# shaneson0/attacking_federate_learning

Measured on AMD Instinct MI355X. Metric: aggregation rounds/sec at N clients x D params (Bulyan), higher is better.
Workload: dtype f32 (Gram: fp16x2 split of every fp32 operand, 3 fp16 MFMAs per block, fp32/fp64 accumulate; <= 2e-7 of |gi||gj| vs f...

## Files before the change

attacking_federate_learning_amd/_native.py:

```python
import ctypes
import os

_HERE = os.path.dirname(os.path.abspath(__file__))
LIB_PATH = os.environ.get('BYZ_LIBRARY') or os.path.join(_HERE, 'libbyzagg.so')

OK, E_INVALID, E_PRECONDITION, E_HIP, E_UNSUPPORTED, E_NO_WINNER, E_COLLECTIVE = 0, -1, -2, -3, -4, -5, -6

KERNELS = ('column_stats', 'gram_tile', 'gram_reduce', 'distances', 'row_sort', 'krum_argmin',
           'bulyan_loop', 'trimmed_mean', 'misc', 'plane_split')

c_i64, c_i32, c_int, c_f32, c_vp = ctypes.c_int64, ctypes.c_int32, ctypes.c_int, ctypes.c_float, ctypes.c_void_p
_P = ctypes.POINTER



class GeomedParams(ctypes.Structure):
    _fields_ = [('nu', ctypes.c_double), ('max_iter', c_i64), ('ftol', ctypes.c_double)]


class CclipParams(ctypes.Structure):
    _fields_ = [('tau', ctypes.c_double), ('iters', c_i64)]


class DncParams(ctypes.Structure):
# ... 90 lines not shown
    'byz_robust_lr_info': [c_vp, _P(c_i64)],
    'byz_robust_lr_host': [c_vp, c_vp, c_i64, c_i64, c_i64, c_vp, c_vp],
    'byz_bucket_means_dev': [c_vp, c_vp, c_i64, c_i64, c_i64, c_vp, c_i64, c_vp, c_i64, c_vp],
    'byz_bucket_means_host': [c_vp, c_vp, c_i64, c_i64, c_vp, c_i64, c_vp],
    'byz_dnc_scores_dev': [c_vp, c_vp, c_i64, c_i64, c_i64, c_vp, c_i64, c_i64, c_vp, c_vp],
    'byz_dnc_select_dev': [c_vp, c_vp, c_i64, c_i64, c_i64, _P(DncParams), c_vp, c_vp, c_vp, c_vp],
    'byz_dnc_dev': [c_vp, c_vp, c_i64, c_i64, c_i64, _P(DncParams), c_vp, c_vp, c_vp, c_vp],
    'byz_dnc_info': [c_vp, _P(c_i64), _P(c_i64)],
    'byz_dnc_host': [c_vp, c_vp, c_i64, c_i64, _P(DncParams), c_vp, c_vp, c_vp, _P(c_i64)],
    'byz_dnc_sharded_dev': [c_vp, c_vp, c_i64, c_i64, c_i64, _P(DncParams), c_vp, c_vp, c_vp, c_vp, c_vp, c_vp, c_vp],
    'byz_timing_enable': [c_vp, c_int],
    'byz_timing_reset': [c_vp],
    'byz_timing_read': [c_vp, c_int, _P(ctypes.c_double), _P(c_i64)],
    'byz_kernel_name': [c_int],
    'byz_selftest_lane_exchange_dev': [c_vp, c_vp, _P(c_i32), c_vp],
}
_RESTYPES = {'byz_last_error': ctypes.c_char_p, 'byz_kernel_name': ctypes.c_char_p, 'byz_ctx_destroy': None}

ALLREDUCE_F64_FN = ctypes.CFUNCTYPE(c_int, c_vp, c_vp, c_i64, c_vp)

EXPORTED_SYMBOLS = tuple(_PROTOTYPES)

_lib = None


class NativeLibraryMissing(RuntimeError):
    pass


def _share_hip_runtime_with_torch():
# ... 43 lines not shown
```

attacking_federate_learning_amd/csrc/api.hip:

```cpp
#include "common.hpp"

#include <cstring>

namespace byz {

static thread_local char g_error[1024] = "";

void set_error(const char* fmt, ...) {
    va_list ap;
    va_start(ap, fmt);
    vsnprintf(g_error, sizeof(g_error), fmt, ap);
    va_end(ap);
}

namespace {

int64_t python_prefix_len(int64_t length, int64_t stop) {
    if (stop >= 0) return stop < length ? stop : length;
    return length + stop > 0 ? length + stop : 0;
}

int enter(byz_ctx* ctx) {
    if (!ctx) {
        set_error("null context");
// ... 1621 lines not shown
        (void)hipEventDestroy(ev.first);
        (void)hipEventDestroy(ev.second);
    }
    slot.pending.clear();
    if (total_ms) *total_ms = slot.total_ms;
    if (launches) *launches = slot.launches;
    return BYZ_OK;
}

int byz_selftest_lane_exchange_dev(byz_ctx* ctx, int32_t* out_dev, int32_t* n_patterns_host, void* stream) {
    BYZ_TRY(enter(ctx));
    BYZ_REQUIRE(out_dev && n_patterns_host, "selftest: bad arguments");
    return launch_lane_selftest(ctx, out_dev, n_patterns_host, as_stream(stream));
}

}
```

attacking_federate_learning_amd/csrc/common.hpp:

```cpp
#pragma once

#include <hip/hip_runtime.h>

#include <cstdarg>
#include <cstdint>
#include <cstdio>
#include <cstdlib>
#include <string>
#include <unordered_map>
#include <vector>

#include "../../include/byzagg.h"

namespace byz {

void set_error(const char* fmt, ...);

#define BYZ_HIP(expr)                                                                       \
    do {                                                                                    \
        hipError_t e_ = (expr);                                                             \
        if (e_ != hipSuccess) {                                                             \
            ::byz::set_error("%s failed: %s (%s:%d)", #expr, hipGetErrorString(e_), __FILE__, \
                             __LINE__);                                                     \
            return BYZ_E_HIP;                                                               \
// ... 69 lines not shown
    int num_cus = 256;
    byz::Buffer gram_partials;
    byz::Buffer gram;
    byz::Buffer tile_order;
    byz::Buffer dup_rep;
    byz::Buffer gram_tickets;
    byz::Buffer gram_planes;
    byz::Buffer gram_chunk_sums;
    byz::Buffer plane_unscale;
    byz::Buffer plane_order;
    byz::Buffer spec_owner;
    byz::Buffer split_redo;
    std::vector<int32_t> plane_order_host;
    int64_t plane_order_T = -1;
    int64_t plane_order_share = 1 * 65536 + 0;
    byz::Buffer row_signature;
    byz::Buffer unique_rows;
    byz::Buffer row_map;
    byz::Buffer gram_compact;
    std::vector<int32_t> tile_order_host;
    int64_t tile_order_T = -1;
    int64_t tile_order_share = 1 * 65536 + 0;
    byz::Buffer tile_owned;
    int64_t row_map_rows = 0;
    byz::Buffer gram_rep;
    byz::Buffer near_pairs;
    byz::Buffer near_sq;
    byz::Buffer near_rows;
    byz::Buffer near_partial;
    int64_t near_pair_capacity = 0;
// ... 151 lines not shown
                         int64_t n, float lr, float z, float* out, hipStream_t stream);
int launch_assemble_row(byz_ctx* ctx, float* row, int64_t n_cols, int64_t n_segments, const float* const* segments,
                        const int64_t* lengths, hipStream_t stream);
int launch_assemble_columns(byz_ctx* ctx, float* G, int64_t n_rows, int64_t n_cols, int64_t ld, int64_t n_segments,
                            const float* const* segments, const int64_t* lengths, hipStream_t stream);
int launch_assemble_rows_again(byz_ctx* ctx, float* G, int64_t n_cols, int64_t ld, int64_t n_clients, int64_t n_segments,
                               hipStream_t stream);
int launch_assemble_rows(byz_ctx* ctx, float* G, int64_t n_cols, int64_t ld, int64_t n_clients, int64_t n_segments,
                         const float* const* segments, const int64_t* lengths, hipStream_t stream);

int launch_gram(byz_ctx* ctx, const float* G, int64_t n_rows, int64_t n_cols, int64_t ld, double* gram,
                hipStream_t stream);
bool gram_planes_enabled();
int launch_gram_planes(byz_ctx* ctx, const float* G, int64_t n_rows, int64_t n_cols, int64_t ld, const int32_t* row_index,
                       double* slabs, int share_count, int share_index, uint8_t* owned_host, bool f16, hipStream_t stream);
int launch_gram_share(byz_ctx* ctx, const float* G, int64_t n_rows, int64_t n_cols, int64_t ld, const int32_t* row_index,
                      int share_count, int share_index, double* gram, hipStream_t stream, bool accumulate = false);
int find_unique_rows(byz_ctx* ctx, const float* G, int64_t n_rows, int64_t n_cols, int64_t ld, hipStream_t stream,
                     int64_t* n_unique_host);
int launch_gram_expand(byz_ctx* ctx, const double* compact, int64_t n_unique, int64_t n_rows, double* gram,
                       hipStream_t stream);
int launch_distances_from_gram(byz_ctx* ctx, const double* gram, int64_t n, float* dist, hipStream_t stream,
                               const float* G, int64_t n_cols, int64_t ld);
int launch_near_pair_sqdist(byz_ctx* ctx, const float* G, int64_t n_cols, int64_t ld, const int32_t* row_index,
                            double* sq_dev, hipStream_t stream);
int launch_near_pair_apply(byz_ctx* ctx, const double* sq_dev, int64_t n, float* dist, hipStream_t stream);

int launch_row_sort(byz_ctx* ctx, const float* dist, int64_t n, int64_t prefix_len, int64_t drop_count,
                    bool want_tables, hipStream_t stream);
int launch_krum_argmin(byz_ctx* ctx, int64_t n, int32_t* winner_dev, hipStream_t stream);
// ... 77 lines not shown
```

attacking_federate_learning_amd/csrc/gram_planes.hip:

```cpp
#include "common.hpp"

#include <cstring>
#include <type_traits>

namespace byz {
namespace {

constexpr int kWgRows = 256;
constexpr int kWgCols = 128;
constexpr int kSlab = 128;
constexpr int kThreads = 512;
constexpr int kFragBytes = 1024;
constexpr int kRowBlocks = (kWgRows + kWgCols) / 32;
constexpr int kChunkCols = 8192;
constexpr int kChunkSteps = kChunkCols / 16;
constexpr int kFlushSteps = 16;
constexpr int kSpareRoundsPercent = 10;

typedef float f32x16 __attribute__((ext_vector_type(16)));
typedef float f32x4 __attribute__((ext_vector_type(4)));
typedef __bf16 bf16x8 __attribute__((ext_vector_type(8)));
typedef _Float16 f16x8 __attribute__((ext_vector_type(8)));
typedef uint32_t u32x4 __attribute__((ext_vector_type(4)));

// ... 518 lines not shown
    }
    asm volatile("s_waitcnt vmcnt(0)" ::: "memory");
    __syncthreads();
    if (tid == 0) {
        __builtin_amdgcn_fence(__ATOMIC_RELEASE, "agent");
        asm volatile("s_waitcnt vmcnt(0)" ::: "memory");
        __hip_atomic_store(tickets + t_list, chunk + 1, __ATOMIC_RELAXED, __HIP_MEMORY_SCOPE_AGENT);
        __hip_atomic_fetch_add(done, 1, __ATOMIC_RELAXED, __HIP_MEMORY_SCOPE_AGENT);
    }
}

template <int NBUF, bool DEFER>
__global__ __launch_bounds__(512, 1) void gram_planes16_kernel(const u32x4* __restrict__ planes, int64_t n_steps,
                                                            const double* __restrict__ unscale, int64_t rows_pad,
                                                            double* __restrict__ partial, int n_tiles,
                                                            const int2* __restrict__ tile_order, int n_chunks,
                                                            int* __restrict__ tickets, int round_size, int run, int t128,
                                                            int slab_live0, int n_blocks32,
                                                            int32_t* __restrict__ device_status,
                                                            float* __restrict__ chunk_sums,
                                                            float* __restrict__ ragged_sums) {
    constexpr int PLANES = 2;
    constexpr int kRbBytes = PLANES * kFragBytes;
    constexpr int kStage = kRowBlocks * kRbBytes;
    constexpr int NW = 8;
    constexpr int kPerWave = kRowBlocks * PLANES / NW;
    constexpr int kSuperFlush = kFlushSteps / 2;
    static_assert(kRowBlocks * PLANES % NW == 0 && NBUF == 6, "ring arithmetic below");
    typedef f16x8 frag_t;
    extern __shared__ __attribute__((aligned(16))) unsigned char lds[];

    const int xcd = blockIdx.x & 7;
    const int seq = blockIdx.x >> 3;
// ... 23 lines not shown
            while (v <= 0) {
                __builtin_amdgcn_s_sleep(1);
                v = __hip_atomic_load(slot, __ATOMIC_RELAXED, __HIP_MEMORY_SCOPE_AGENT);
            }
            claimed_round = v - 1;
        }
        __syncthreads();
    }
    const int unit = __builtin_amdgcn_readfirstlane(claimed_round * run + seq % run);
    const int chunk = __builtin_amdgcn_readfirstlane(unit / n_tiles);
    if (chunk >= n_chunks) {
        if (threadIdx.x == 0) __hip_atomic_fetch_add(done, 1, __ATOMIC_RELAXED, __HIP_MEMORY_SCOPE_AGENT);
        return;
    }
    const int t_list = unit - chunk * n_tiles;
    const int2 tt = tile_order[t_list];
    const int bi = __builtin_amdgcn_readfirstlane(tt.x);
    const int tj = __builtin_amdgcn_readfirstlane(tt.y);

    const int tid = threadIdx.x;
    const int lane = tid & 63;
    const int wave = __builtin_amdgcn_readfirstlane(tid >> 6);
    const int wr = wave >> 1, wc = wave & 1;
    const int ti = 2 * bi + wr / 2;
    const int row_in_slab = (wr % 2) * 64;
    unsigned live_blocks = 0;
    if (tj <= ti && ti < t128 && n_blocks32 < 0) {
        live_blocks = 15u;
    } else if (tj <= ti && ti < t128) {
#pragma unroll
        for (int m = 0; m < 2; ++m)
#pragma unroll
            for (int n = 0; n < 2; ++n) {
                const int rblk = ti * 4 + row_in_slab / 32 + m, cblk = tj * 4 + wc * 2 + n;
                if (rblk < n_blocks32 && cblk <= rblk) live_blocks |= 1u << (m * 2 + n);
            }
    }
    const bool live_wave = live_blocks != 0;

    const int step0 = chunk * kChunkSteps;
    int n_stages = static_cast<int>(n_steps) - step0;
    if (n_stages > kChunkSteps) n_stages = kChunkSteps;
    const int n_super = n_stages / 2;

    int64_t piece_off[kPerWave];
#pragma unroll
    for (int i = 0; i < kPerWave; ++i) {
        const int q = wave + NW * i;
        const int rbl = q / PLANES, piece = q % PLANES;
        const int64_t rb = rbl < 8 ? static_cast<int64_t>(bi) * 8 + rbl : static_cast<int64_t>(tj) * 4 + (rbl - 8);
        piece_off[i] = (((rb * n_steps + step0) * PLANES + piece) * 64) * 16;
    }
    const unsigned char* lane_base = reinterpret_cast<const unsigned char*>(planes) + lane * 16;
    auto dma_piece = [&](int s, int i) __attribute__((always_inline)) {
        unsigned char* dst = lds + (s % NBUF) * kStage + wave * kFragBytes;
        __builtin_amdgcn_global_load_lds(
            (const __attribute__((address_space(1))) void*)(lane_base + piece_off[i] + static_cast<int64_t>(s) * (PLANES * kFragBytes)),
            (__attribute__((address_space(3))) void*)(dst + i * NW * kFragBytes), 16, 0, 0);
    };
    auto dma = [&](int s) __attribute__((always_inline)) {
#pragma unroll
        for (int i = 0; i < kPerWave; ++i) dma_piece(s, i);
    };

    f32x4 acc[4][4], acc2[4][4];
// ... 10 lines not shown
    const int lane_in_image = (lane & 15) + 32 * ((lane >> 4) & 1);
    const int pair_half = lane >> 5;
    auto frag_at = [&](int sp, int rb32, int h, int p) __attribute__((always_inline)) -> frag_t {
        const unsigned char* at = lds + (2 * (sp % (NBUF / 2)) + pair_half) * kStage + rb32 * kRbBytes + p * kFragBytes +
                                  (lane_in_image + 16 * h) * 16;
        return *reinterpret_cast<const frag_t*>(at);
    };
    struct AFrags { frag_t v[2][4]; };
    struct BFrags { frag_t v[2][2]; };
    auto read_a = [&](int sp, AFrags& a, auto mask_c) __attribute__((always_inline)) {
        constexpr unsigned MASK = decltype(mask_c)::value;
#pragma unroll
        for (int p = 0; p < 2; ++p)
#pragma unroll
            for (int m = 0; m < 4; ++m)
                if (((MASK >> ((m / 2) * 2)) & 3u) != 0) a.v[p][m] = frag_at(sp, 2 * wr + m / 2, m % 2, p);
    };
    auto read_b = [&](int sp, int half, BFrags& b, auto mask_c) __attribute__((always_inline)) {
        constexpr unsigned MASK = decltype(mask_c)::value;
#pragma unroll
        for (int p = 0; p < 2; ++p)
#pragma unroll
            for (int n = 0; n < 2; ++n) b.v[p][n] = frag_at(sp, 8 + 2 * wc + half, n, p);
        (void)MASK;
    };
    auto multiply_half = [&](const AFrags& a, const BFrags& b, auto half_c, auto mask_c) __attribute__((always_inline)) {
        constexpr unsigned MASK = decltype(mask_c)::value;
        constexpr int HALF = decltype(half_c)::value;
        constexpr int pa[3] = {1, 0, 0};
        constexpr int pb[3] = {0, 1, 0};
#pragma unroll
        for (int t = 0; t < 3; ++t)
#pragma unroll
            for (int m = 0; m < 4; ++m)
#pragma unroll
                for (int n = 0; n < 2; ++n)
                    if (((MASK >> ((m / 2) * 2 + HALF)) & 1u) != 0)
                        acc[m][2 * HALF + n] = __builtin_amdgcn_mfma_f32_16x16x32_f16(a.v[pa[t]][m], b.v[pb[t]][n], acc[m][2 * HALF + n], 0, 0, 0);
// ... 48 lines not shown
                    read_a(sp + 1, an, mask_c);
                    if ((MASK & 5u) != 0) read_b(sp + 1, 0, b0, mask_c);
                }
                if ((MASK & 10u) != 0) multiply_half(a, b1, h1, mask_c);
                flush(sp);
            }
        };
        auto super8 = [&](int sp, AFrags& a, AFrags& an, auto pos_c) __attribute__((always_inline)) {
            constexpr int POS = decltype(pos_c)::value;
            constexpr bool FRESH = POS == 0, FLUSHING = POS == 7;
            constexpr int pa[3] = {1, 0, 0};
            constexpr int pb[3] = {0, 1, 0};
            const f32x4 zero4 = {0.0f, 0.0f, 0.0f, 0.0f};
#pragma unroll
            for (int g = 0; g < 4; ++g) {
                b1.v[g / 2][g % 2] = frag_at(sp, 8 + 2 * wc + 1, g % 2, g / 2);
#pragma unroll
                for (int q = 6 * g; q < 6 * g + 6; ++q) {
                    const int t = q / 8, m = (q % 8) / 2, n = q % 2;
                    acc[m][n] = __builtin_amdgcn_mfma_f32_16x16x32_f16(a.v[pa[t]][m], b0.v[pb[t]][n], (FRESH && t == 0) ? zero4 : acc[m][n], 0, 0, 0);
                }
                __builtin_amdgcn_sched_barrier(0);
            }
            wait_vmcnt<2 * kPerWave>();
            asm volatile("s_waitcnt lgkmcnt(0)\n\ts_barrier" ::: "memory");
#pragma unroll
            for (int g = 0; g < 6; ++g) {
                dma_piece(2 * sp + NBUF + g / 3, g % 3);
#pragma unroll
                for (int r = 2 * g; r < 2 * g + 2; ++r) {
                    if (r < 8) an.v[r / 4][r % 4] = frag_at(sp + 1, 2 * wr + (r % 4) / 2, (r % 4) % 2, r / 4);
                    else b0.v[(r - 8) / 2][(r - 8) % 2] = frag_at(sp + 1, 8 + 2 * wc + 0, (r - 8) % 2, (r - 8) / 2);
                }
#pragma unroll
                for (int q = 4 * g; q < 4 * g + 4; ++q) {
                    const int t = q / 8, m = (q % 8) / 2, n = q % 2;
                    acc[m][2 + n] = __builtin_amdgcn_mfma_f32_16x16x32_f16(a.v[pa[t]][m], b1.v[pb[t]][n], (FRESH && t == 0) ? zero4 : acc[m][2 + n], 0, 0, 0);
                }
                if constexpr (FLUSHING) {
#pragma unroll
                    for (int b = (8 * g) / 6; b < (8 * (g + 1)) / 6; ++b)
#pragma unroll
                        for (int e = 0; e < 4; ++e) acc2[b / 2][b % 2][e] += acc[b / 2][b % 2][e];
                }
                __builtin_amdgcn_sched_barrier(0);
            }
            if constexpr (FLUSHING) {
// ... 33 lines not shown
            super(sp + 1, a1, a0);
        }
        if (sp < n_super) super(sp, a0, a1);
    };
    switch (live_blocks) {
        case 0u: k_loop(std::integral_constant<unsigned, 0u>{}); break;
        case 1u: k_loop(std::integral_constant<unsigned, 1u>{}); break;
        case 3u: k_loop(std::integral_constant<unsigned, 3u>{}); break;
        case 13u: k_loop(std::integral_constant<unsigned, 13u>{}); break;
        default: live_blocks = 15u; k_loop(std::integral_constant<unsigned, 15u>{}); break;
    }
    auto block_live = [&](int m, int n) __attribute__((always_inline)) { return ((live_blocks >> ((m / 2) * 2 + n / 2)) & 1u) != 0; };

    if constexpr (DEFER) {
        if (live_wave) {
            const int sel = wr / 2;
            const bool unflushed = (n_super % kSuperFlush) != 0;
            float* out = chunk_sums + ((static_cast<int64_t>(chunk) * n_tiles + t_list) * 2 + sel) * (kSlab * kSlab);
            float* rag = ragged_sums + (static_cast<int64_t>(t_list) * 2 + sel) * (kSlab * kSlab);
#pragma unroll
            for (int m = 0; m < 4; ++m)
#pragma unroll
                for (int n = 0; n < 4; ++n) {
                    if (!block_live(m, n)) continue;
                    const int j = wc * 64 + 16 * n + (lane & 15);
#pragma unroll
                    for (int e = 0; e < 4; ++e) {
                        const int i = row_in_slab + 16 * m + 4 * (lane >> 4) + e;
                        out[i * kSlab + j] = acc2[m][n][e];
                        if (unflushed) rag[i * kSlab + j] = acc[m][n][e];
                    }
                }
        }
        __syncthreads();
        if (tid == 0) __hip_atomic_fetch_add(done, 1, __ATOMIC_RELAXED, __HIP_MEMORY_SCOPE_AGENT);
        return;
    }
    bool lost = false;
    if (chunk > 0) {
        if (tid == 0) {
// ... 1 lines not shown
            while (__hip_atomic_load(tickets + t_list, __ATOMIC_RELAXED, __HIP_MEMORY_SCOPE_AGENT) != chunk) {
                __builtin_amdgcn_s_sleep(8);
                if (++spins > (1u << 26)) {
                    lost = true;
                    break;
                }
            }
            __builtin_amdgcn_fence(__ATOMIC_ACQUIRE, "agent");
        }
        lost = __syncthreads_or(lost ? 1 : 0) != 0;
    }
    if (lost) {
        if (tid == 0) atomicOr(device_status, kStatusLostTicket);
    } else if (live_wave) {
        const bool slab_live = chunk > 0 || slab_live0 != 0;
        double* out = partial + (static_cast<int64_t>(ti) * (ti + 1) / 2 + tj) * (kSlab * kSlab);
        const double* un = unscale + static_cast<int64_t>(chunk) * rows_pad;
#pragma unroll
        for (int m = 0; m < 4; ++m)
#pragma unroll
            for (int n = 0; n < 4; ++n) {
                if (!block_live(m, n)) continue;
                const int j = wc * 64 + 16 * n + (lane & 15);
                const double uj = un[static_cast<int64_t>(tj) * kSlab + j];
#pragma unroll
                for (int e = 0; e < 4; ++e) {
                    const int i = row_in_slab + 16 * m + 4 * (lane >> 4) + e;
                    double v = static_cast<double>(acc2[m][n][e]);
                    v += static_cast<double>(acc[m][n][e]);
                    v *= un[static_cast<int64_t>(ti) * kSlab + i] * uj;
                    if (slab_live) v += out[i * kSlab + j];
                    out[i * kSlab + j] = v;
                }
            }
    }
    asm volatile("s_waitcnt vmcnt(0)" ::: "memory");
    __syncthreads();
    if (tid == 0) {
        __builtin_amdgcn_fence(__ATOMIC_RELEASE, "agent");
        asm volatile("s_waitcnt vmcnt(0)" ::: "memory");
        __hip_atomic_store(tickets + t_list, chunk + 1, __ATOMIC_RELAXED, __HIP_MEMORY_SCOPE_AGENT);
        __hip_atomic_fetch_add(done, 1, __ATOMIC_RELAXED, __HIP_MEMORY_SCOPE_AGENT);
    }
}

constexpr int kReduceRun = 8;
__global__ __launch_bounds__(256) void chunk_reduce_kernel(const float* __restrict__ chunk_sums, const float* __restrict__ ragged_sums,
                                                           int n_tiles, int n_chunks, int ragged_chunk,
                                                           const int2* __restrict__ tile_order, const double* __restrict__ unscale,
                                                           int64_t rows_pad, double* __restrict__ partial, int slab_live0,
                                                           int t128, int n_blocks32) {
    typedef double f64x4 __attribute__((ext_vector_type(4)));
    const int t_list = blockIdx.x >> 1, sel = blockIdx.x & 1;
    const int2 tt = tile_order[t_list];
    const int ti = 2 * tt.x + sel, tj = tt.y;
    if (!(tj <= ti && ti < t128)) return;
    double* out = partial + (static_cast<int64_t>(ti) * (ti + 1) / 2 + tj) * (kSlab * kSlab);
    const int64_t slab_stride = static_cast<int64_t>(n_tiles) * 2 * (kSlab * kSlab);
    const float* in = chunk_sums + (static_cast<int64_t>(t_list) * 2 + sel) * (kSlab * kSlab);
    const float* rag = ragged_sums + (static_cast<int64_t>(t_list) * 2 + sel) * (kSlab * kSlab);
    const int i = static_cast<int>(blockIdx.y) * 32 + (threadIdx.x >> 3), j = (threadIdx.x & 7) * 4;
    for (int jb = 0; jb < kSlab; jb += 32) {
        const int jj = jb + j;
        if (n_blocks32 >= 0) {
            const int rblk = ti * 4 + (i >> 5), cblk = tj * 4 + (jj >> 5);
            if (!(rblk < n_blocks32 && cblk <= rblk)) continue;
        }
        const int idx = i * kSlab + jj;
        f64x4 v = {0.0, 0.0, 0.0, 0.0};
        bool live = slab_live0 != 0;
        if (live) v = *reinterpret_cast<const f64x4*>(out + idx);
        for (int c0 = 0; c0 < n_chunks; c0 += kReduceRun) {
            f32x4 p[kReduceRun];
            double ui[kReduceRun];
            f64x4 uj[kReduceRun];
// ... 19 lines not shown
                for (int e = 0; e < 4; ++e) {
                    q[e] *= ui[k] * uj[k][e];
                    v[e] = live ? q[e] + v[e] : q[e];
                }
                live = true;
            }
        }
        *reinterpret_cast<f64x4*>(out + idx) = v;
    }
}

}

bool gram_planes_enabled() { return env_int("BYZ_GRAM_PLANES", 1) != 0; }

int launch_gram_planes(byz_ctx* ctx, const float* G, int64_t n_rows, int64_t n_cols, int64_t ld, const int32_t* row_index,
                       double* slabs, int share_count, int share_index, uint8_t* owned_host, bool f16, hipStream_t stream) {
    const int64_t t128 = ceil_div(n_rows, kSlab);
    const int64_t t256 = ceil_div(t128, 2);
    const int64_t rows_pad = t256 * kWgRows;
    const int64_t order_key = static_cast<int64_t>(f16 ? 1 : 0) * (1ll << 40) + share_count * 65536 + share_index;
    if (ctx->plane_order_T != t128 || ctx->plane_order_share != order_key) {
        ctx->plane_order_host.clear();
        int64_t position = 0;
        auto push = [&](int64_t bi, int64_t tj) {
            if (position++ % share_count != share_index) return;
            ctx->plane_order_host.push_back(static_cast<int32_t>(bi));
            ctx->plane_order_host.push_back(static_cast<int32_t>(tj));
        };
        if (f16) {
            for (int64_t b0 = 0; b0 < t256; b0 += 4)
                for (int64_t tj = 0; tj < t128 && tj <= 2 * (b0 + 3) + 1; ++tj)
                    for (int64_t bi = b0; bi < b0 + 4 && bi < t256; ++bi)
                        if (tj <= 2 * bi + 1) push(bi, tj);
        } else {
            const int64_t S = ceil_div(t128, 8);
            for (int64_t I = 0; I < S; ++I)
                for (int64_t J = 0; J <= I; ++J)
                    for (int64_t bi = I * 4; bi < I * 4 + 4 && bi < t256; ++bi)
                        for (int64_t tj = J * 8; tj < J * 8 + 8 && tj <= 2 * bi + 1 && tj < t128; ++tj) push(bi, tj);
        }
        BYZ_TRY(ctx->plane_order.ensure(ctx->plane_order_host.size() * sizeof(int32_t) + 16));
        BYZ_HIP(hipMemcpyAsync(ctx->plane_order.ptr, ctx->plane_order_host.data(),
                               ctx->plane_order_host.size() * sizeof(int32_t), hipMemcpyHostToDevice, stream));
        BYZ_HIP(hipStreamSynchronize(stream));
        ctx->plane_order_T = t128;
        ctx->plane_order_share = order_key;
    }
    const int64_t n_tiles = static_cast<int64_t>(ctx->plane_order_host.size() / 2);
    if (owned_host != nullptr)
        for (int64_t t = 0; t < n_tiles; ++t) {
            const int64_t bi = ctx->plane_order_host[2 * t], tj = ctx->plane_order_host[2 * t + 1];
            for (int64_t ti = 2 * bi; ti < 2 * bi + 2 && ti < t128; ++ti)
                if (tj <= ti) owned_host[ti * (ti + 1) / 2 + tj] = 1;
        }
    if (n_tiles == 0) return BYZ_OK;

    const int n_planes = f16 ? 2 : 3;
    size_t free_b = 0, total_b = 0;
    BYZ_HIP(hipMemGetInfo(&free_b, &total_b));
    int64_t budget = static_cast<int64_t>(env_int("BYZ_GRAM_PLANE_MB", 16384)) << 20;
    const int64_t have = static_cast<int64_t>(ctx->gram_planes.bytes);
    if (budget > have + static_cast<int64_t>(free_b / 2)) budget = have + static_cast<int64_t>(free_b / 2);
    int64_t chunks_per_sc = budget / (rows_pad * 2 * n_planes * kChunkCols);
    const int64_t chunks_total = ceil_div(n_cols, kChunkCols);
    if (chunks_per_sc > chunks_total) chunks_per_sc = chunks_total;
    if (chunks_per_sc < 1) {
        set_error("gram: no room for one 8192-column chunk of 16-bit planes (%lld rows)", (long long)rows_pad);
        return BYZ_E_HIP;
    }
    const int64_t n_sc = ceil_div(chunks_total, chunks_per_sc);
    chunks_per_sc = ceil_div(chunks_total, n_sc);
    const int64_t sc_cols = chunks_per_sc * kChunkCols;
    BYZ_TRY(ctx->gram_planes.ensure(static_cast<size_t>(rows_pad) * 2 * n_planes * sc_cols));
    double* unscale = nullptr;
    if (f16) {
        BYZ_TRY(ctx->plane_unscale.ensure(static_cast<size_t>(rows_pad) * chunks_per_sc * sizeof(double)));
        unscale = ctx->plane_unscale.as<double>();
    }
    u32x4* planes = ctx->gram_planes.as<u32x4>();
    bool defer = f16 && env_int("BYZ_GRAM_DEFER", 1) != 0;
    float* chunk_sums = nullptr;
    float* ragged_sums = nullptr;
    if (defer) {
        const size_t per_chunk = static_cast<size_t>(n_tiles) * 2 * kSlab * kSlab * sizeof(float);
        const size_t want = per_chunk * static_cast<size_t>(chunks_per_sc + 1);
        size_t free_now = 0, total_now = 0;
        BYZ_HIP(hipMemGetInfo(&free_now, &total_now));
        if (want > ctx->gram_chunk_sums.bytes && want - ctx->gram_chunk_sums.bytes > free_now / 2) defer = false;
    }
    if (defer) {
        const size_t per_chunk = static_cast<size_t>(n_tiles) * 2 * kSlab * kSlab * sizeof(float);
        BYZ_TRY(ctx->gram_chunk_sums.ensure(per_chunk * static_cast<size_t>(chunks_per_sc + 1)));
        chunk_sums = ctx->gram_chunk_sums.as<float>();
        ragged_sums = chunk_sums + (per_chunk / sizeof(float)) * static_cast<size_t>(chunks_per_sc);
    }
    auto kernel16 = defer ? &gram_planes16_kernel<6, true> : &gram_planes16_kernel<6, false>;
    const void* kernel = f16 ? reinterpret_cast<const void*>(kernel16) : reinterpret_cast<const void*>(&gram_planes_kernel<4>);
    const size_t lds_bytes = static_cast<size_t>(f16 ? 6 : 4) * kRowBlocks * n_planes * kFragBytes;
    BYZ_HIP(allow_dynamic_lds(ctx, kernel, static_cast<int>(lds_bytes)));
    const int round_size = env_int("BYZ_GRAM_ROUND", ctx->num_cus / 8);
    const int run = round_size > 0 ? round_size : ctx->num_cus / 8;
    const int n_blocks32 = env_int("BYZ_GRAM_BLOCK_SKIP", 1) != 0 ? static_cast<int>(ceil_div(n_rows, 32)) : -1;
    const int64_t per_xcd = ceil_div(n_tiles, 8);
    for (int64_t sc = 0; sc < n_sc; ++sc) {
        const int64_t k0 = sc * sc_cols;
        const int64_t cols = n_cols - k0 < sc_cols ? n_cols - k0 : sc_cols;
        const int64_t n_steps = ceil_div(cols, 32) * 2;
        const int64_t n_chunks = ceil_div(n_steps, kChunkSteps);
        {
            KernelTimer t(ctx, BYZ_K_PLANE_SPLIT, stream);
            if (f16) {
                const dim3 grid(static_cast<unsigned>(n_chunks), static_cast<unsigned>(rows_pad / 32));
                if (env_int("BYZ_GRAM_SPLIT_TWO_PASS", 0) != 0) {
                    plane_split_f16_kernel<<<grid, 256, 0, stream>>>(G, n_rows, n_cols, ld, row_index, k0, n_steps, planes,
                                                                     unscale, rows_pad, nullptr);
                } else {
                    const int64_t pairs = n_chunks * (rows_pad / 32);
// ... 17 lines not shown
            int64_t rounds_per_xcd = 0;
            if (f16) {
                rounds_per_xcd = ceil_div(ceil_div(n_tiles * n_chunks, run), 8);
                rounds_per_xcd += rounds_per_xcd * kSpareRoundsPercent / 100;
            }
            const int64_t grid = f16 ? 8 * run * rounds_per_xcd : 8 * per_xcd * n_chunks;
            const size_t ticket_ints = static_cast<size_t>(n_tiles + 9 + 8 * rounds_per_xcd);
            BYZ_TRY(ctx->gram_tickets.ensure(ticket_ints * sizeof(int)));
            int* tickets = ctx->gram_tickets.as<int>();
            BYZ_HIP(hipMemsetAsync(tickets, 0, ticket_ints * sizeof(int), stream));
            KernelTimer t(ctx, BYZ_K_GRAM, stream);
            if (grid > 0x7fffffff) {
                set_error("gram: grid too large");
                return BYZ_E_UNSUPPORTED;
            }
            const int2* tile_order = ctx->plane_order.as<int2>();
            const int slab_live0 = sc > 0 ? 1 : 0;
            if (!f16) {
                gram_planes_kernel<4><<<static_cast<unsigned>(grid), kThreads, lds_bytes, stream>>>(
                    planes, n_steps, slabs, static_cast<int>(n_tiles), tile_order, static_cast<int>(n_chunks), tickets,
                    round_size, static_cast<int>(t128), slab_live0, n_blocks32, device_status_word(ctx));
            } else {
                kernel16<<<static_cast<unsigned>(grid), kThreads, lds_bytes, stream>>>(
                    planes, n_steps, unscale, rows_pad, slabs, static_cast<int>(n_tiles), tile_order, static_cast<int>(n_chunks),
                    tickets, round_size, run, static_cast<int>(t128), slab_live0, n_blocks32, device_status_word(ctx),
                    chunk_sums, ragged_sums);
            }
            BYZ_TRY(check_launch("gram_planes_kernel"));
        }
        if (defer) {
            KernelTimer t(ctx, BYZ_K_GRAM_REDUCE, stream);
            const int ragged_chunk = (n_steps % kChunkSteps) % kFlushSteps != 0 ? static_cast<int>(n_chunks) - 1 : -1;
            chunk_reduce_kernel<<<dim3(static_cast<unsigned>(2 * n_tiles), 4), 256, 0, stream>>>(
                chunk_sums, ragged_sums, static_cast<int>(n_tiles), static_cast<int>(n_chunks), ragged_chunk,
                ctx->plane_order.as<int2>(), unscale, rows_pad, slabs, sc > 0 ? 1 : 0, static_cast<int>(t128), n_blocks32);
            BYZ_TRY(check_launch("chunk_reduce_kernel"));
        }
    }
    return BYZ_OK;
}

}
```

include/byzagg.h:

```cpp
#ifndef BYZAGG_H
#define BYZAGG_H

#include <stdint.h>

#ifdef __cplusplus
extern "C" {
#endif

#define BYZ_ABI_VERSION 1

enum {
    BYZ_OK = 0,
    BYZ_E_INVALID = -1,
    BYZ_E_PRECONDITION = -2,
    BYZ_E_HIP = -3,
    BYZ_E_UNSUPPORTED = -4,
    BYZ_E_NO_WINNER = -5,
    BYZ_E_COLLECTIVE = -6
};

typedef struct byz_ctx byz_ctx;

int byz_abi_version(void);
const char* byz_last_error(void);
// ... 259 lines not shown
                 const int64_t* columns_host, float* out_host, int32_t* good_host, int64_t* kept_host);

enum {
    BYZ_K_COLUMN_STATS = 0, BYZ_K_GRAM = 1, BYZ_K_GRAM_REDUCE = 2, BYZ_K_DISTANCES = 3,
    BYZ_K_ROW_SORT = 4, BYZ_K_KRUM_ARGMIN = 5, BYZ_K_BULYAN_LOOP = 6, BYZ_K_TRIMMED_MEAN = 7,
    BYZ_K_MISC = 8, BYZ_K_PLANE_SPLIT = 9, BYZ_K_COUNT = 10
};
int byz_timing_enable(byz_ctx* ctx, int on);
int byz_timing_reset(byz_ctx* ctx);
int byz_timing_read(byz_ctx* ctx, int kernel, double* total_ms, int64_t* launches);
const char* byz_kernel_name(int kernel);

int byz_selftest_lane_exchange_dev(byz_ctx* ctx, int32_t* out_dev, int32_t* n_patterns_host,
                                   void* stream);

#ifdef __cplusplus
}
#endif
#endif
```

Baseline: 1.975.

## Drive fp16 Gram kernel from per-wave unit table with packed diagonal units

Replaces the fp16 Gram kernel's (bi,tj) tile list with a host-built table of GramUnits. Each unit holds 12 row-block indices plus per-wave LDS slots, live-block masks, sum slots and output slabs. Diagonal tiles that used to leave waves idle are packed, up to three per unit, into shared units. Deferred chunk sums are indexed by slot rather than by two per tile, so wasted MFMA waves and empty reduction blocks on the triangular diagonal are meant to go away. The cost is a larger table per unit, more scalar loads, and more complex host bookkeeping, including a fallback when defer is disabled.

```diff
diff --git a/attacking_federate_learning_amd/_native.py b/attacking_federate_learning_amd/_native.py
--- a/attacking_federate_learning_amd/_native.py
+++ b/attacking_federate_learning_amd/_native.py
@@ -128,6 +128,7 @@
     'byz_timing_read': [c_vp, c_int, _P(ctypes.c_double), _P(c_i64)],
     'byz_kernel_name': [c_int],
     'byz_selftest_lane_exchange_dev': [c_vp, c_vp, _P(c_i32), c_vp],
+    'byz_gram_unit_table': [c_i64, _P(c_i32), c_i64, _P(c_i64)],
 }
 _RESTYPES = {'byz_last_error': ctypes.c_char_p, 'byz_kernel_name': ctypes.c_char_p, 'byz_ctx_destroy': None}
 
diff --git a/attacking_federate_learning_amd/csrc/api.hip b/attacking_federate_learning_amd/csrc/api.hip
--- a/attacking_federate_learning_amd/csrc/api.hip
+++ b/attacking_federate_learning_amd/csrc/api.hip
@@ -1659,4 +1659,18 @@
     return launch_lane_selftest(ctx, out_dev, n_patterns_host, as_stream(stream));
 }
 
-}
+int byz_gram_unit_table(int64_t n_rows, int32_t* units_host, int64_t capacity_units, int64_t* n_units) {
+    static_assert(kGramUnitWords == BYZ_GRAM_UNIT_WORDS, "the header describes GramUnit");
+    if (n_rows < 1 || n_rows > 32767ll * 128 || !n_units || capacity_units < 0) return BYZ_E_INVALID;
+    std::vector<GramUnit> units;
+    std::vector<int32_t> slot_slab;
+    build_gram_units(ceil_div(n_rows, 128), ceil_div(n_rows, 32), true, 1, 0, units, slot_slab);
+    *n_units = static_cast<int64_t>(units.size());
+    if (units_host) {
+        const int64_t count = *n_units < capacity_units ? *n_units : capacity_units;
+        std::memcpy(units_host, units.data(), static_cast<size_t>(count) * sizeof(GramUnit));
+    }
+    return BYZ_OK;
+}
+
+}
diff --git a/attacking_federate_learning_amd/csrc/common.hpp b/attacking_federate_learning_amd/csrc/common.hpp
--- a/attacking_federate_learning_amd/csrc/common.hpp
+++ b/attacking_federate_learning_amd/csrc/common.hpp
@@ -107,6 +107,8 @@
     std::vector<int32_t> plane_order_host;
     int64_t plane_order_T = -1;
     int64_t plane_order_share = 1 * 65536 + 0;
+    int64_t plane_order_blocks = -2;
+    int64_t plane_units = 0, plane_sum_slots = 0;
     byz::Buffer row_signature;
     byz::Buffer unique_rows;
     byz::Buffer row_map;
@@ -288,6 +290,17 @@
 bool gram_planes_enabled();
 int launch_gram_planes(byz_ctx* ctx, const float* G, int64_t n_rows, int64_t n_cols, int64_t ld, const int32_t* row_index,
                        double* slabs, int share_count, int share_index, uint8_t* owned_host, bool f16, hipStream_t stream);
+struct GramUnitWave {
+    uint32_t where;
+    int32_t sum_slot, slab;
+};
+struct GramUnit {
+    int32_t rb[12];
+    GramUnitWave wave[8];
+};
+constexpr int kGramUnitWords = static_cast<int>(sizeof(GramUnit) / sizeof(int32_t));
+void build_gram_units(int64_t t128, int64_t n_blocks32, bool diagonal_units, int share_count, int share_index,
+                      std::vector<GramUnit>& units, std::vector<int32_t>& slot_slab);
 int launch_gram_share(byz_ctx* ctx, const float* G, int64_t n_rows, int64_t n_cols, int64_t ld, const int32_t* row_index,
                       int share_count, int share_index, double* gram, hipStream_t stream, bool accumulate = false);
 int find_unique_rows(byz_ctx* ctx, const float* G, int64_t n_rows, int64_t n_cols, int64_t ld, hipStream_t stream,
diff --git a/attacking_federate_learning_amd/csrc/gram_planes.hip b/attacking_federate_learning_amd/csrc/gram_planes.hip
--- a/attacking_federate_learning_amd/csrc/gram_planes.hip
+++ b/attacking_federate_learning_amd/csrc/gram_planes.hip
@@ -556,9 +556,9 @@
 __global__ __launch_bounds__(512, 1) void gram_planes16_kernel(const u32x4* __restrict__ planes, int64_t n_steps,
                                                             const double* __restrict__ unscale, int64_t rows_pad,
                                                             double* __restrict__ partial, int n_tiles,
-                                                            const int2* __restrict__ tile_order, int n_chunks,
-                                                            int* __restrict__ tickets, int round_size, int run, int t128,
-                                                            int slab_live0, int n_blocks32,
+                                                            const GramUnit* __restrict__ units, int n_chunks,
+                                                            int* __restrict__ tickets, int round_size, int run,
+                                                            int slab_live0, int n_sum_slots,
                                                             int32_t* __restrict__ device_status,
                                                             float* __restrict__ chunk_sums,
                                                             float* __restrict__ ragged_sums) {
@@ -612,28 +612,18 @@
         return;
     }
     const int t_list = unit - chunk * n_tiles;
-    const int2 tt = tile_order[t_list];
-    const int bi = __builtin_amdgcn_readfirstlane(tt.x);
-    const int tj = __builtin_amdgcn_readfirstlane(tt.y);
+    const GramUnit* __restrict__ my_unit = units + t_list;
 
     const int tid = threadIdx.x;
     const int lane = tid & 63;
     const int wave = __builtin_amdgcn_readfirstlane(tid >> 6);
-    const int wr = wave >> 1, wc = wave & 1;
-    const int ti = 2 * bi + wr / 2;
-    const int row_in_slab = (wr % 2) * 64;
-    unsigned live_blocks = 0;
-    if (tj <= ti && ti < t128 && n_blocks32 < 0) {
-        live_blocks = 15u;
-    } else if (tj <= ti && ti < t128) {
-#pragma unroll
-        for (int m = 0; m < 2; ++m)
-#pragma unroll
-            for (int n = 0; n < 2; ++n) {
-                const int rblk = ti * 4 + row_in_slab / 32 + m, cblk = tj * 4 + wc * 2 + n;
-                if (rblk < n_blocks32 && cblk <= rblk) live_blocks |= 1u << (m * 2 + n);
-            }
-    }
+    const unsigned where = static_cast<unsigned>(__builtin_amdgcn_readfirstlane(my_unit->wave[wave].where));
+    const int a_slot = static_cast<int>(where & 0xffu);
+    const int b_slot = static_cast<int>((where >> 8) & 0xffu);
+    unsigned live_blocks = (where >> 16) & 0xffu;
+    const int row_in_slab = static_cast<int>((where >> 24) & 1u) * 64;
+    const int col_in_slab = static_cast<int>((where >> 25) & 1u) * 64;
+    const int sum_slot = __builtin_amdgcn_readfirstlane(my_unit->wave[wave].sum_slot);
     const bool live_wave = live_blocks != 0;
 
     const int step0 = chunk * kChunkSteps;
@@ -646,7 +636,7 @@
     for (int i = 0; i < kPerWave; ++i) {
         const int q = wave + NW * i;
         const int rbl = q / PLANES, piece = q % PLANES;
-        const int64_t rb = rbl < 8 ? static_cast<int64_t>(bi) * 8 + rbl : static_cast<int64_t>(tj) * 4 + (rbl - 8);
+        const int64_t rb = __builtin_amdgcn_readfirstlane(my_unit->rb[rbl]);
         piece_off[i] = (((rb * n_steps + step0) * PLANES + piece) * 64) * 16;
     }
     const unsigned char* lane_base = reinterpret_cast<const unsigned char*>(planes) + lane * 16;
@@ -687,14 +677,14 @@
         for (int p = 0; p < 2; ++p)
 #pragma unroll
             for (int m = 0; m < 4; ++m)
-                if (((MASK >> ((m / 2) * 2)) & 3u) != 0) a.v[p][m] = frag_at(sp, 2 * wr + m / 2, m % 2, p);
+                if (((MASK >> ((m / 2) * 2)) & 3u) != 0) a.v[p][m] = frag_at(sp, a_slot + m / 2, m % 2, p);
     };
     auto read_b = [&](int sp, int half, BFrags& b, auto mask_c) __attribute__((always_inline)) {
         constexpr unsigned MASK = decltype(mask_c)::value;
 #pragma unroll
         for (int p = 0; p < 2; ++p)
 #pragma unroll
-            for (int n = 0; n < 2; ++n) b.v[p][n] = frag_at(sp, 8 + 2 * wc + half, n, p);
+            for (int n = 0; n < 2; ++n) b.v[p][n] = frag_at(sp, b_slot + half, n, p);
         (void)MASK;
     };
     auto multiply_half = [&](const AFrags& a, const BFrags& b, auto half_c, auto mask_c) __attribute__((always_inline)) {
@@ -773,7 +763,7 @@
             const f32x4 zero4 = {0.0f, 0.0f, 0.0f, 0.0f};
 #pragma unroll
             for (int g = 0; g < 4; ++g) {
-                b1.v[g / 2][g % 2] = frag_at(sp, 8 + 2 * wc + 1, g % 2, g / 2);
+                b1.v[g / 2][g % 2] = frag_at(sp, b_slot + 1, g % 2, g / 2);
 #pragma unroll
                 for (int q = 6 * g; q < 6 * g + 6; ++q) {
                     const int t = q / 8, m = (q % 8) / 2, n = q % 2;
@@ -788,8 +778,8 @@
                 dma_piece(2 * sp + NBUF + g / 3, g % 3);
 #pragma unroll
                 for (int r = 2 * g; r < 2 * g + 2; ++r) {
-                    if (r < 8) an.v[r / 4][r % 4] = frag_at(sp + 1, 2 * wr + (r % 4) / 2, (r % 4) % 2, r / 4);
-                    else b0.v[(r - 8) / 2][(r - 8) % 2] = frag_at(sp + 1, 8 + 2 * wc + 0, (r - 8) % 2, (r - 8) / 2);
+                    if (r < 8) an.v[r / 4][r % 4] = frag_at(sp + 1, a_slot + (r % 4) / 2, (r % 4) % 2, r / 4);
+                    else b0.v[(r - 8) / 2][(r - 8) % 2] = frag_at(sp + 1, b_slot, (r - 8) % 2, (r - 8) / 2);
                 }
 #pragma unroll
                 for (int q = 4 * g; q < 4 * g + 4; ++q) {
@@ -853,16 +843,15 @@
 
     if constexpr (DEFER) {
         if (live_wave) {
-            const int sel = wr / 2;
             const bool unflushed = (n_super % kSuperFlush) != 0;
-            float* out = chunk_sums + ((static_cast<int64_t>(chunk) * n_tiles + t_list) * 2 + sel) * (kSlab * kSlab);
-            float* rag = ragged_sums + (static_cast<int64_t>(t_list) * 2 + sel) * (kSlab * kSlab);
+            float* out = chunk_sums + (static_cast<int64_t>(chunk) * n_sum_slots + sum_slot) * (kSlab * kSlab);
+            float* rag = ragged_sums + static_cast<int64_t>(sum_slot) * (kSlab * kSlab);
 #pragma unroll
             for (int m = 0; m < 4; ++m)
 #pragma unroll
                 for (int n = 0; n < 4; ++n) {
                     if (!block_live(m, n)) continue;
-                    const int j = wc * 64 + 16 * n + (lane & 15);
+                    const int j = col_in_slab + 16 * n + (lane & 15);
 #pragma unroll
                     for (int e = 0; e < 4; ++e) {
                         const int i = row_in_slab + 16 * m + 4 * (lane >> 4) + e;
@@ -894,6 +883,8 @@
         if (tid == 0) atomicOr(device_status, kStatusLostTicket);
     } else if (live_wave) {
         const bool slab_live = chunk > 0 || slab_live0 != 0;
+        const int slab = __builtin_amdgcn_readfirstlane(my_unit->wave[wave].slab);
+        const int ti = slab & 0xffff, tj = slab >> 16;
         double* out = partial + (static_cast<int64_t>(ti) * (ti + 1) / 2 + tj) * (kSlab * kSlab);
         const double* un = unscale + static_cast<int64_t>(chunk) * rows_pad;
 #pragma unroll
@@ -901,7 +892,7 @@
 #pragma unroll
             for (int n = 0; n < 4; ++n) {
                 if (!block_live(m, n)) continue;
-                const int j = wc * 64 + 16 * n + (lane & 15);
+                const int j = col_in_slab + 16 * n + (lane & 15);
                 const double uj = un[static_cast<int64_t>(tj) * kSlab + j];
 #pragma unroll
                 for (int e = 0; e < 4; ++e) {
@@ -926,19 +917,19 @@
 
 constexpr int kReduceRun = 8;
 __global__ __launch_bounds__(256) void chunk_reduce_kernel(const float* __restrict__ chunk_sums, const float* __restrict__ ragged_sums,
-                                                           int n_tiles, int n_chunks, int ragged_chunk,
-                                                           const int2* __restrict__ tile_order, const double* __restrict__ unscale,
+                                                           int n_sum_slots, int n_chunks, int ragged_chunk,
+                                                           const int2* __restrict__ slot_slab, const double* __restrict__ unscale,
                                                            int64_t rows_pad, double* __restrict__ partial, int slab_live0,
-                                                           int t128, int n_blocks32) {
+                                                           int n_blocks32) {
     typedef double f64x4 __attribute__((ext_vector_type(4)));
-    const int t_list = blockIdx.x >> 1, sel = blockIdx.x & 1;
-    const int2 tt = tile_order[t_list];
-    const int ti = 2 * tt.x + sel, tj = tt.y;
-    if (!(tj <= ti && ti < t128)) return;
+    const int slot = blockIdx.x;
+    const int2 tt = slot_slab[slot];
+    const int ti = tt.x, tj = tt.y;
+    if (ti < 0) return;
     double* out = partial + (static_cast<int64_t>(ti) * (ti + 1) / 2 + tj) * (kSlab * kSlab);
-    const int64_t slab_stride = static_cast<int64_t>(n_tiles) * 2 * (kSlab * kSlab);
-    const float* in = chunk_sums + (static_cast<int64_t>(t_list) * 2 + sel) * (kSlab * kSlab);
-    const float* rag = ragged_sums + (static_cast<int64_t>(t_list) * 2 + sel) * (kSlab * kSlab);
+    const int64_t slab_stride = static_cast<int64_t>(n_sum_slots) * (kSlab * kSlab);
+    const float* in = chunk_sums + static_cast<int64_t>(slot) * (kSlab * kSlab);
+    const float* rag = ragged_sums + static_cast<int64_t>(slot) * (kSlab * kSlab);
     const int i = static_cast<int>(blockIdx.y) * 32 + (threadIdx.x >> 3), j = (threadIdx.x & 7) * 4;
     for (int jb = 0; jb < kSlab; jb += 32) {
         const int jj = jb + j;
@@ -988,46 +979,155 @@
 
 bool gram_planes_enabled() { return env_int("BYZ_GRAM_PLANES", 1) != 0; }
 
+void build_gram_units(int64_t t128, int64_t n_blocks32, bool diagonal_units, int share_count, int share_index,
+                      std::vector<GramUnit>& units, std::vector<int32_t>& slot_slab) {
+    units.clear();
+    slot_slab.clear();
+    const int64_t t256 = ceil_div(t128, 2);
+    auto live_mask = [&](int64_t ti, int64_t tj, int row64, int col64) -> uint32_t {
+        if (!(tj <= ti && ti < t128)) return 0u;
+        if (n_blocks32 < 0) return 15u;
+        uint32_t mask = 0;
+        for (int m = 0; m < 2; ++m)
+            for (int n = 0; n < 2; ++n) {
+                const int64_t rblk = ti * 4 + row64 * 2 + m, cblk = tj * 4 + col64 * 2 + n;
+                if (rblk < n_blocks32 && cblk <= rblk) mask |= 1u << (m * 2 + n);
+            }
+        return mask;
+    };
+    auto set_wave = [&](GramUnit& u, int wave, int a_slot, int b_slot, int64_t ti, int64_t tj, int row64, int col64,
+                        int64_t sum_slot) {
+        const uint32_t mask = live_mask(ti, tj, row64, col64);
+        GramUnitWave& w = u.wave[wave];
+        w.where = static_cast<uint32_t>(a_slot) | static_cast<uint32_t>(b_slot) << 8 | mask << 16 |
+                  static_cast<uint32_t>(row64) << 24 | static_cast<uint32_t>(col64) << 25;
+        w.sum_slot = mask != 0 ? static_cast<int32_t>(sum_slot) : 0;
+        w.slab = mask != 0 ? static_cast<int32_t>(ti | tj << 16) : 0;
+    };
+    auto slab_slot = [](int64_t ti, int64_t tj) { return ti * (ti + 1) / 2 + tj; };
+    int64_t position = 0;
+    auto plain = [&](int64_t bi, int64_t tj, bool d1) {
+        if (position++ % share_count != share_index) return;
+        const int64_t t_list = static_cast<int64_t>(units.size());
+        GramUnit u{};
+        for (int s = 0; s < 12; ++s) u.rb[s] = static_cast<int32_t>(s < 8 ? bi * 8 + s : tj * 4 + (s - 8));
+        for (int wave = 0; wave < 8; ++wave) {
+            const int wr = wave / 2, wc = wave % 2;
+            const int64_t ti = 2 * bi + wr / 2;
+            set_wave(u, wave, 2 * wr, 8 + 2 * wc, ti, tj, wr % 2, wc, diagonal_units ? slab_slot(ti, tj) : 2 * t_list + wr / 2);
+        }
+        if (d1) set_wave(u, 1, 4, 4, 2 * bi + 1, 2 * bi + 1, 0, 0, slab_slot(2 * bi + 1, 2 * bi + 1));
+        units.push_back(u);
+        if (!diagonal_units)
+            for (int sel = 0; sel < 2; ++sel) {
+                const int64_t ti = 2 * bi + sel;
+                const bool live = tj <= ti && ti < t128;
+                slot_slab.push_back(static_cast<int32_t>(live ? ti : -1));
+                slot_slab.push_back(static_cast<int32_t>(live ? tj : -1));
+            }
+    };
+    auto d2 = [&](int64_t first, int64_t count) {
+        static const int partial_wave[3] = {3, 7, 5};
+        GramUnit u{};
+        for (int s = 0; s < 12; ++s) u.rb[s] = static_cast<int32_t>(first * 8 + 4);
+        for (int64_t k = 0; k < count; ++k) {
+            const int64_t bi = first + k, t = 2 * bi + 1;
+            for (int s = 0; s < 4; ++s) u.rb[4 * k + s] = static_cast<int32_t>(bi * 8 + 4 + s);
+            set_wave(u, static_cast<int>(k), static_cast<int>(4 * k + 2), static_cast<int>(4 * k), t, t, 1, 0, slab_slot(t, t));
+            set_wave(u, partial_wave[k], static_cast<int>(4 * k + 2), static_cast<int>(4 * k + 2), t, t, 1, 1, slab_slot(t, t));
+        }
+        units.push_back(u);
+    };
+    const int64_t full_blocks = t128 / 2;
+    for (int64_t b0 = 0; b0 < t256; b0 += 4)
+        for (int64_t tj = 0; tj < t128 && tj <= 2 * (b0 + 3) + 1; ++tj)
+            for (int64_t bi = b0; bi < b0 + 4 && bi < t256; ++bi) {
+                if (tj > 2 * bi + 1) continue;
+                if (!diagonal_units) {
+                    plain(bi, tj, false);
+                } else if (tj == 2 * bi + 1) {
+                    if (bi % 3 == 2 || bi == full_blocks - 1) d2(bi - bi % 3, bi % 3 + 1);
+                } else {
+                    plain(bi, tj, tj == 2 * bi);
+                }
+            }
+    if (diagonal_units)
+        for (int64_t ti = 0; ti < t128; ++ti)
+            for (int64_t tj = 0; tj <= ti; ++tj) {
+                slot_slab.push_back(static_cast<int32_t>(ti));
+                slot_slab.push_back(static_cast<int32_t>(tj));
+            }
+}
+
 int launch_gram_planes(byz_ctx* ctx, const float* G, int64_t n_rows, int64_t n_cols, int64_t ld, const int32_t* row_index,
                        double* slabs, int share_count, int share_index, uint8_t* owned_host, bool f16, hipStream_t stream) {
     const int64_t t128 = ceil_div(n_rows, kSlab);
     const int64_t t256 = ceil_div(t128, 2);
     const int64_t rows_pad = t256 * kWgRows;
-    const int64_t order_key = static_cast<int64_t>(f16 ? 1 : 0) * (1ll << 40) + share_count * 65536 + share_index;
-    if (ctx->plane_order_T != t128 || ctx->plane_order_share != order_key) {
-        ctx->plane_order_host.clear();
-        int64_t position = 0;
-        auto push = [&](int64_t bi, int64_t tj) {
-            if (position++ % share_count != share_index) return;
-            ctx->plane_order_host.push_back(static_cast<int32_t>(bi));
-            ctx->plane_order_host.push_back(static_cast<int32_t>(tj));
-        };
+    bool defer = f16 && env_int("BYZ_GRAM_DEFER", 1) != 0;
+    const int n_blocks32 = env_int("BYZ_GRAM_BLOCK_SKIP", 1) != 0 ? static_cast<int>(ceil_div(n_rows, 32)) : -1;
+    auto ensure_list = [&](bool diagonal_units) -> int {
+        const int64_t order_key = static_cast<int64_t>((f16 ? 1 : 0) + (diagonal_units ? 2 : 0)) * (1ll << 40) + share_count * 65536 + share_index;
+        const int64_t blocks_key = f16 ? n_blocks32 : -2;
+        if (ctx->plane_order_T != t128 || ctx->plane_order_share != order_key || ctx->plane_order_blocks != blocks_key) {
+            ctx->plane_order_host.clear();
+            if (f16) {
+                if (t128 > 0x7fff) {
+                    set_error("gram: more than 32767 slabs per side");
+                    return BYZ_E_UNSUPPORTED;
+                }
+                std::vector<GramUnit> units;
+                std::vector<int32_t> slot_slab;
+                build_gram_units(t128, n_blocks32, diagonal_units, share_count, share_index, units, slot_slab);
+                ctx->plane_units = static_cast<int64_t>(units.size());
+                ctx->plane_sum_slots = static_cast<int64_t>(slot_slab.size() / 2);
+                ctx->plane_order_host.resize(units.size() * kGramUnitWords);
+                if (!units.empty()) std::memcpy(ctx->plane_order_host.data(), units.data(), units.size() * sizeof(GramUnit));
+                ctx->plane_order_host.insert(ctx->plane_order_host.end(), slot_slab.begin(), slot_slab.end());
+            } else {
+                int64_t position = 0;
+                auto push = [&](int64_t bi, int64_t tj) {
+                    if (position++ % share_count != share_index) return;
+                    ctx->plane_order_host.push_back(static_cast<int32_t>(bi));
+                    ctx->plane_order_host.push_back(static_cast<int32_t>(tj));
+                };
+                const int64_t S = ceil_div(t128, 8);
+                for (int64_t I = 0; I < S; ++I)
+                    for (int64_t J = 0; J <= I; ++J)
+                        for (int64_t bi = I * 4; bi < I * 4 + 4 && bi < t256; ++bi)
+                            for (int64_t tj = J * 8; tj < J * 8 + 8 && tj <= 2 * bi + 1 && tj < t128; ++tj) push(bi, tj);
+                ctx->plane_units = static_cast<int64_t>(ctx->plane_order_host.size() / 2);
+                ctx->plane_sum_slots = 0;
+            }
+            BYZ_TRY(ctx->plane_order.ensure(ctx->plane_order_host.size() * sizeof(int32_t) + 16));
+            BYZ_HIP(hipMemcpyAsync(ctx->plane_order.ptr, ctx->plane_order_host.data(),
+                                   ctx->plane_order_host.size() * sizeof(int32_t), hipMemcpyHostToDevice, stream));
+            BYZ_HIP(hipStreamSynchronize(stream));
+            ctx->plane_order_T = t128;
+            ctx->plane_order_share = order_key;
+            ctx->plane_order_blocks = blocks_key;
+        }
+        return BYZ_OK;
+    };
+    const bool diagonal_units = defer && share_count == 1 && n_blocks32 >= 0;
+    BYZ_TRY(ensure_list(diagonal_units));
+    int64_t n_tiles = ctx->plane_units;
+    int64_t n_sum_slots = ctx->plane_sum_slots;
+    const int32_t* slot_slab_host = ctx->plane_order_host.data() + n_tiles * kGramUnitWords;
+    if (owned_host != nullptr) {
         if (f16) {
-            for (int64_t b0 = 0; b0 < t256; b0 += 4)
-                for (int64_t tj = 0; tj < t128 && tj <= 2 * (b0 + 3) + 1; ++tj)
-                    for (int64_t bi = b0; bi < b0 + 4 && bi < t256; ++bi)
-                        if (tj <= 2 * bi + 1) push(bi, tj);
+            for (int64_t s = 0; s < n_sum_slots; ++s) {
+                const int64_t ti = slot_slab_host[2 * s], tj = slot_slab_host[2 * s + 1];
+                if (ti >= 0) owned_host[ti * (ti + 1) / 2 + tj] = 1;
+            }
         } else {
-            const int64_t S = ceil_div(t128, 8);
-            for (int64_t I = 0; I < S; ++I)
-                for (int64_t J = 0; J <= I; ++J)
-                    for (int64_t bi = I * 4; bi < I * 4 + 4 && bi < t256; ++bi)
-                        for (int64_t tj = J * 8; tj < J * 8 + 8 && tj <= 2 * bi + 1 && tj < t128; ++tj) push(bi, tj);
-        }
-        BYZ_TRY(ctx->plane_order.ensure(ctx->plane_order_host.size() * sizeof(int32_t) + 16));
-        BYZ_HIP(hipMemcpyAsync(ctx->plane_order.ptr, ctx->plane_order_host.data(),
-                               ctx->plane_order_host.size() * sizeof(int32_t), hipMemcpyHostToDevice, stream));
-        BYZ_HIP(hipStreamSynchronize(stream));
-        ctx->plane_order_T = t128;
-        ctx->plane_order_share = order_key;
-    }
-    const int64_t n_tiles = static_cast<int64_t>(ctx->plane_order_host.size() / 2);
-    if (owned_host != nullptr)
-        for (int64_t t = 0; t < n_tiles; ++t) {
-            const int64_t bi = ctx->plane_order_host[2 * t], tj = ctx->plane_order_host[2 * t + 1];
-            for (int64_t ti = 2 * bi; ti < 2 * bi + 2 && ti < t128; ++ti)
-                if (tj <= ti) owned_host[ti * (ti + 1) / 2 + tj] = 1;
-        }
+            for (int64_t t = 0; t < n_tiles; ++t) {
+                const int64_t bi = ctx->plane_order_host[2 * t], tj = ctx->plane_order_host[2 * t + 1];
+                for (int64_t ti = 2 * bi; ti < 2 * bi + 2 && ti < t128; ++ti)
+                    if (tj <= ti) owned_host[ti * (ti + 1) / 2 + tj] = 1;
+            }
+        }
+    }
     if (n_tiles == 0) return BYZ_OK;
 
     const int n_planes = f16 ? 2 : 3;
@@ -1053,18 +1153,22 @@
         unscale = ctx->plane_unscale.as<double>();
     }
     u32x4* planes = ctx->gram_planes.as<u32x4>();
-    bool defer = f16 && env_int("BYZ_GRAM_DEFER", 1) != 0;
     float* chunk_sums = nullptr;
     float* ragged_sums = nullptr;
     if (defer) {
-        const size_t per_chunk = static_cast<size_t>(n_tiles) * 2 * kSlab * kSlab * sizeof(float);
+        const size_t per_chunk = static_cast<size_t>(n_sum_slots) * kSlab * kSlab * sizeof(float);
         const size_t want = per_chunk * static_cast<size_t>(chunks_per_sc + 1);
         size_t free_now = 0, total_now = 0;
         BYZ_HIP(hipMemGetInfo(&free_now, &total_now));
         if (want > ctx->gram_chunk_sums.bytes && want - ctx->gram_chunk_sums.bytes > free_now / 2) defer = false;
+        if (!defer && diagonal_units) {
+            BYZ_TRY(ensure_list(false));
+            n_tiles = ctx->plane_units;
+            n_sum_slots = ctx->plane_sum_slots;
+        }
     }
     if (defer) {
-        const size_t per_chunk = static_cast<size_t>(n_tiles) * 2 * kSlab * kSlab * sizeof(float);
+        const size_t per_chunk = static_cast<size_t>(n_sum_slots) * kSlab * kSlab * sizeof(float);
         BYZ_TRY(ctx->gram_chunk_sums.ensure(per_chunk * static_cast<size_t>(chunks_per_sc + 1)));
         chunk_sums = ctx->gram_chunk_sums.as<float>();
         ragged_sums = chunk_sums + (per_chunk / sizeof(float)) * static_cast<size_t>(chunks_per_sc);
@@ -1075,7 +1179,6 @@
     BYZ_HIP(allow_dynamic_lds(ctx, kernel, static_cast<int>(lds_bytes)));
     const int round_size = env_int("BYZ_GRAM_ROUND", ctx->num_cus / 8);
     const int run = round_size > 0 ? round_size : ctx->num_cus / 8;
-    const int n_blocks32 = env_int("BYZ_GRAM_BLOCK_SKIP", 1) != 0 ? static_cast<int>(ceil_div(n_rows, 32)) : -1;
     const int64_t per_xcd = ceil_div(n_tiles, 8);
     for (int64_t sc = 0; sc < n_sc; ++sc) {
         const int64_t k0 = sc * sc_cols;
@@ -1123,26 +1226,26 @@
                 set_error("gram: grid too large");
                 return BYZ_E_UNSUPPORTED;
             }
-            const int2* tile_order = ctx->plane_order.as<int2>();
             const int slab_live0 = sc > 0 ? 1 : 0;
             if (!f16) {
                 gram_planes_kernel<4><<<static_cast<unsigned>(grid), kThreads, lds_bytes, stream>>>(
-                    planes, n_steps, slabs, static_cast<int>(n_tiles), tile_order, static_cast<int>(n_chunks), tickets,
+                    planes, n_steps, slabs, static_cast<int>(n_tiles), ctx->plane_order.as<int2>(), static_cast<int>(n_chunks), tickets,
                     round_size, static_cast<int>(t128), slab_live0, n_blocks32, device_status_word(ctx));
             } else {
                 kernel16<<<static_cast<unsigned>(grid), kThreads, lds_bytes, stream>>>(
-                    planes, n_steps, unscale, rows_pad, slabs, static_cast<int>(n_tiles), tile_order, static_cast<int>(n_chunks),
-                    tickets, round_size, run, static_cast<int>(t128), slab_live0, n_blocks32, device_status_word(ctx),
-                    chunk_sums, ragged_sums);
+                    planes, n_steps, unscale, rows_pad, slabs, static_cast<int>(n_tiles), ctx->plane_order.as<GramUnit>(),
+                    static_cast<int>(n_chunks), tickets, round_size, run, slab_live0, static_cast<int>(n_sum_slots),
+                    device_status_word(ctx), chunk_sums, ragged_sums);
             }
             BYZ_TRY(check_launch("gram_planes_kernel"));
         }
         if (defer) {
             KernelTimer t(ctx, BYZ_K_GRAM_REDUCE, stream);
             const int ragged_chunk = (n_steps % kChunkSteps) % kFlushSteps != 0 ? static_cast<int>(n_chunks) - 1 : -1;
-            chunk_reduce_kernel<<<dim3(static_cast<unsigned>(2 * n_tiles), 4), 256, 0, stream>>>(
-                chunk_sums, ragged_sums, static_cast<int>(n_tiles), static_cast<int>(n_chunks), ragged_chunk,
-                ctx->plane_order.as<int2>(), unscale, rows_pad, slabs, sc > 0 ? 1 : 0, static_cast<int>(t128), n_blocks32);
+            const int2* slot_slab = reinterpret_cast<const int2*>(ctx->plane_order.as<GramUnit>() + n_tiles);
+            chunk_reduce_kernel<<<dim3(static_cast<unsigned>(n_sum_slots), 4), 256, 0, stream>>>(
+                chunk_sums, ragged_sums, static_cast<int>(n_sum_slots), static_cast<int>(n_chunks), ragged_chunk, slot_slab,
+                unscale, rows_pad, slabs, sc > 0 ? 1 : 0, n_blocks32);
             BYZ_TRY(check_launch("chunk_reduce_kernel"));
         }
     }
diff --git a/include/byzagg.h b/include/byzagg.h
--- a/include/byzagg.h
+++ b/include/byzagg.h
@@ -297,6 +297,9 @@
 int byz_selftest_lane_exchange_dev(byz_ctx* ctx, int32_t* out_dev, int32_t* n_patterns_host,
                                    void* stream);
 
+#define BYZ_GRAM_UNIT_WORDS 36
+int byz_gram_unit_table(int64_t n_rows, int32_t* units_host, int64_t capacity_units, int64_t* n_units);
+
 #ifdef __cplusplus
 }
 #endif
```

New measurement: 2.004 (median of 6 runs). 1.01x the previous value.
